# leopard-ai/betty

Measured on AMD Instinct MI355X. Metric: hypergradient-steps/sec (CG K=20, 10M inner params), higher is better.
Workload: dtype f32

## Files before the change

### betty_amd/_native.py

```python
from __future__ import annotations

import ctypes
import os
from ctypes import POINTER, c_char_p, c_double, c_float, c_int, c_int32, c_int64, c_size_t, c_void_p

_HERE = os.path.dirname(os.path.abspath(__file__))
LIB_PATH = os.environ.get("BHG_LIB") or os.path.join(_HERE, "csrc", "libbhg.so")
AB_LIB_PATH = os.environ.get("BHG_AB_LIB") or os.path.join(_HERE, "csrc", "libbhg_ab.so")

BHG_CHUNK_ELEMS = 4096
BHG_FLAT_ALIGN = 64
BHG_CG_AUTO, BHG_CG_STREAM, BHG_CG_RESIDENT = 0, 1, 2
BHG_CG_GLOBAL_CHAIN, BHG_CG_GLOBAL_UPDATE, BHG_CG_GLOBAL_DOTS = 0, 1, 2
BHG_CG_FX_BEGIN, BHG_CG_FX_CHAIN, BHG_CG_FX_GRAM, BHG_CG_FX_END = 0, 1, 2, 3


class NativeLibraryError(RuntimeError):
    """libbhg.so is missing or a call into it failed."""


class Chunk(ctypes.Structure):

    _fields_ = [
        ("flat_off", c_int64),
# ... 156 lines not shown
    "bhg_mlp_fx_slab_floats": (c_size_t, [POINTER(Mlp)]),
    "bhg_mlp_fx_scal_doubles": (c_size_t, [POINTER(Mlp)]),
    "bhg_mlp_cg_fx_phase": (
        c_int,
        [POINTER(Mlp), _PP, c_int, c_int, c_int, c_int, c_int, c_void_p, c_void_p, c_void_p, c_float, c_float, c_void_p, c_size_t,
         c_void_p, c_size_t, c_void_p],
    ),
    "bhg_mlp_neumann_fx_phase": (
        c_int,
        [POINTER(Mlp), _PP, c_int, c_int, c_int, c_int, c_int, c_void_p, c_void_p, c_void_p, c_float, c_float, c_void_p, c_size_t,
         c_void_p, c_size_t, c_void_p],
    ),
    "bhg_mlp_cg_mixed_coeff": (c_int, [POINTER(Mlp), c_void_p, c_void_p, c_float, c_void_p, c_size_t, c_void_p]),
    "bhg_mlp_timeout_flag_dev": (c_void_p, [POINTER(Mlp), c_void_p]),
    "bhg_mlp_head_j_dev": (c_void_p, [POINTER(Mlp), c_void_p, POINTER(c_int), POINTER(c_int)]),
    "bhg_mlp_stage_batch": (c_int, [POINTER(Mlp), c_void_p, c_void_p, c_void_p, c_void_p]),
    "bhg_mlp_supports_packed_prepare": (c_int, [POINTER(Mlp)]),
    "bhg_mlp_forward_packed": (c_int, [POINTER(Mlp), _PP, c_void_p, c_void_p, c_void_p, c_size_t, c_void_p]),
    "bhg_mlp_backward_packed": (c_int, [POINTER(Mlp), c_void_p, c_void_p, c_size_t, c_void_p]),
    "bhg_mwn_max_hidden": (c_int, []),
    "bhg_mlp_fd_ws_bytes": (c_size_t, [POINTER(c_int), c_int, c_int]),
    "bhg_mlp_fd_forward": (
        c_int,
        [c_void_p, c_void_p, c_int, POINTER(c_int), c_int, _PP, _PP, c_void_p, c_int, c_void_p, c_void_p, c_void_p, c_size_t, c_void_p],
    ),
    "bhg_mwn_fd_vjp": (
        c_int,
        [c_void_p, c_void_p, c_int, c_void_p, c_void_p, c_void_p, c_void_p, c_int, c_void_p, c_int, c_void_p, c_void_p, c_void_p, c_void_p,
         c_void_p],
    ),
# ... 172 lines not shown
```

### betty_amd/csrc/bhg_common.hpp

```cpp
#pragma once
#include <hip/hip_runtime.h>
#include <stdint.h>
#include <stddef.h>
#include <stdio.h>
#include <string.h>

#include "bhg.h"

namespace bhg {

constexpr int kThreads = 256;
constexpr int kWaves = kThreads / 64;
constexpr int kChunk = BHG_CHUNK_ELEMS;
constexpr int kVecPerThread = kChunk / (kThreads * 4);
constexpr int kMaxBlocks = 1024;
constexpr int kInlineT = 32;
constexpr int kWriterT = 448;

constexpr size_t kWsScal = 0;
constexpr size_t kWsPartP = 128;
constexpr size_t kWsPartR = kWsPartP + 8 * kMaxBlocks;
constexpr size_t kWsBarrier = kWsPartR + 16 * kMaxBlocks;
constexpr size_t kWsTables = kWsBarrier + 256;
inline size_t ws_bytes(int T) {
  size_t b = kWsTables + 4 * sizeof(void*) * (size_t)(T > 0 ? T : 0);
  return (b + 255) & ~(size_t)255;
}

enum { S_RR_OLD = 0, S_PHP = 1, S_ALPHA = 2, S_RR_NEW = 3, S_BETA = 4, S_PP = 5 , S_ALPHA_RING = 10 ,
       S_NPART0 = 8  };

#define BHG_DBG_KEYS(X)                                                                                                      \
  X(mlp_wsk) X(mlp_wsk_maxk) X(mlp_wsk_depth) X(mlp_wsk_lds) X(wsl_depth) X(no_nt_slabs) X(gemm_no_xpose) X(mlp_no_fast)      \
  X(mlp_tn) X(split_target) X(split_cap) X(mlp_no_head) X(gram_ksplit) X(gram_kchunk) X(proj_graw_split) X(mlp_proj)         \
  X(mlp_hoist) X(hoist_wgs) X(proj_step_alone) X(mlp_no_side) X(mlp_no_fuse) X(mlp_no_outer_all) X(neumann_side)             \
  X(hoist_staged_mink) X(proj_alpha_alone) X(proj_small_alone) X(outer_order_by_work) X(outer_no_pre) X(outer_stagger)       \
  X(mlp_no_fused_solve) X(cg_eager_p) X(cg_x_every_iter) X(neumann_p_every_iter) X(head_no_prefetch) X(cg_spin_limit)        \
  X(packed_chain) X(packed_depth) X(packed_gram) X(proj_max_ratio) X(proj_ws_cap_mb) X(alpha_in_hoist) X(graw_v2) X(wskp_ragged) X(pstep_v2) X(pstep_unroll) X(rnew_in_graw) X(graw_cols) X(lin_first) X(lin_prio) X(lin_nub) X(lin_order) X(lin_update_next) X(lin_withhold_beta) X(neumann_vnew) X(cg_rhs_direct) X(packed_prepare) X(lin_deep) X(graw_kloop) X(lin_update_in_head) X(xcd_pairs) X(headu_head_first) X(fx_ksplit) X(head_j) X(head_j_tile)
enum DbgKey : int {
#define BHG_DBG_ENUM(n) DBG_##n,
  BHG_DBG_KEYS(BHG_DBG_ENUM)
#undef BHG_DBG_ENUM
  DBG_COUNT
};
constexpr int kDbgUnset = INT32_MIN;
#ifdef BHG_AB
extern int g_dbg[DBG_COUNT];
inline bool dbg_is_set(DbgKey k) { return g_dbg[k] != kDbgUnset; }
inline int dbg(DbgKey k, int dflt) { return g_dbg[k] == kDbgUnset ? dflt : g_dbg[k]; }
#else
constexpr bool dbg_is_set(DbgKey) { return false; }
constexpr int dbg(DbgKey, int dflt) { return dflt; }
#endif
// ... 210 lines not shown
```

### betty_amd/csrc/bhg_mlp.hip

```cpp
#include <stdlib.h>


#include "bhg_common.hpp"
#include "bhg_mlp_headj.hpp"

#ifdef BHG_STAMPS
namespace bhg { __device__ unsigned long long* d_stamps = nullptr; }
#endif

namespace bhg {
namespace {
#include "mlp/gemm.inc"

#include "mlp/outer.inc"

#include "mlp/scalars.inc"

#include "mlp/head.inc"

#include "mlp/wsk.inc"

#include "mlp/wskp.inc"

inline int wsk_mode(int chain_mode, int unfused_hint) {
// ... 469 lines not shown
  int nRR, nT2;
  float* hoist;
  double* part_dot; double* pscal;
  double* part_raw;
  double* part_graw;
  float* pb0[2];
  float* pb1[2];
  unsigned long long* gran;
  float* Wf[BHG_MLP_MAX_LAYERS];
  float* Wb[BHG_MLP_MAX_LAYERS];
  float* hpk[BHG_MLP_MAX_LAYERS];
  float* dpk[BHG_MLP_MAX_LAYERS];
  float* Rhp[BHG_MLP_MAX_LAYERS];
  float* Rdp[BHG_MLP_MAX_LAYERS];
  float* hj_J; float* hj_Ap; int nT2j;
  size_t bytes;
};
inline bool headj_shape_ok(const bhg_mlp* m, const HoistPlan& hp) {
  return hp.ok && hp.lin_ok && m->L == 4 && m->dims[m->L] <= 12 && m->dims[m->L - 1] <= 512 && m->Bp == 128;
}
inline int headj_rows(int rows_valid, int C) { return (rows_valid * C + 31) & ~31; }
void carve_fused_ws(const bhg_mlp* m, void* base, FusedWs* w) {
  memset(w, 0, sizeof(*w));
  const bool head = use_head(m);
  int nrr = bias_blocks(m);
  for (int l = 0; l < m->L; ++l) nrr += outer_blocks(m, l, head);
  w->nRR = nrr;
  size_t off = 0;
  auto take = [&](size_t bytes) { void* p = base ? static_cast<char*>(base) + off : nullptr; off += (bytes + 255) & ~(size_t)255; return p; };
  w->partT1 = static_cast<double*>(take(sizeof(double) * m->Bp));
  w->partT2h = static_cast<double*>(take(sizeof(double) * m->Bp));
  w->partPP = static_cast<double*>(take(sizeof(double) * kMaxBlocks));
  w->partRR[0] = static_cast<double*>(take(sizeof(double) * 3 * nrr));
  w->partRR[1] = static_cast<double*>(take(sizeof(double) * 3 * nrr));
  int nt2 = 0;
  for (int l = 1; l + 1 < m->L; ++l) { w->t2_off[l] = nt2; nt2 += reduce_blocks(m->Bp * m->dims[l], m->dims[l]); }
// ... 19 lines not shown
    for (int l = 0; l + 1 < L; ++l) {
      w->hpk[l] = static_cast<float*>(take(sizeof(float) * Bp * m->dims[l]));
      if (l + 2 < L) w->Rhp[l] = static_cast<float*>(take(sizeof(float) * Bp * m->dims[l + 1]));
      if (l >= 1) {
        w->Wf[l] = static_cast<float*>(take(sizeof(float) * (size_t)m->dims[l + 1] * m->dims[l]));
        w->Wb[l] = static_cast<float*>(take(sizeof(float) * (size_t)m->dims[l + 1] * m->dims[l]));
        w->dpk[l] = static_cast<float*>(take(sizeof(float) * Bp * m->dims[l + 1]));
        w->Rdp[l] = static_cast<float*>(take(sizeof(float) * Bp * m->dims[l + 1]));
      }
    }
  }
  if (hj) {
    const size_t rj = (size_t)headj_rows(m->Bp, m->dims[m->L]);
    w->hj_J = static_cast<float*>(take(sizeof(float) * rj * m->dims[m->L - 2]));
    w->hj_Ap = static_cast<float*>(take(sizeof(float) * rj * m->dims[m->L - 1]));
  }
  w->bytes = off;
}

bool graw_single_on(bool packed, int Bp) { return packed && dbg(DBG_packed_gram, 1) != 0 && dbg(DBG_graw_v2, 1) != 0 && graw_batch_ok(Bp); }
bool rnew_keys_on() { return dbg(DBG_proj_small_alone, 0) == 0 && dbg(DBG_alpha_in_hoist, 1) != 0 && dbg(DBG_rnew_in_graw, 1) != 0; }

int pack_operands(const bhg_mlp* m, const FusedWs& w, hipStream_t st, bool weights_only = false) {
  PackArgs g{};
  int blk = 0;
  auto add = [&](const float* X, float* Xp, int R, int K, int kind) {
    if (g.n >= kPackMax) return false;
    g.p[g.n] = {X, Xp, R, K, kind};
    g.blk0[g.n] = blk;
    blk += pack_blocks(g.p[g.n]);
// ... 16 lines not shown
  BHG_HIP_CHECK(hipGetLastError());
  return BHG_OK;
}

int build_head_j(const bhg_mlp* m, const FusedWs& w, hipStream_t st) {
  const int L = m->L, C = m->dims[L], K = m->dims[L - 1], N = m->dims[L - 2], RA = headj_rows(m->B, C);
  BHG_REQUIRE(w.nT2j > 0 && w.hj_J && w.hj_Ap && w.Wb[L - 2], "the head_j form was planned for a net it cannot take");
  if (int rc = launch_headj_pack(m->W[L - 1], m->mask[L - 2], w.hj_Ap, m->B, C, K, RA, st)) return rc;
  WskpBuilder wb;
  WskpProb q{};
  q.Ap = w.hj_Ap; q.Bq = w.Wb[L - 2]; q.RA = RA; q.RB = N; q.K = K; q.B = m->B * C; q.nsplit = 1;
  q.out = w.hj_J;
  wb.add(q);
  wb.launch(st);
  BHG_HIP_CHECK(hipGetLastError());
  return BHG_OK;
}

#include "mlp/solve_plan.inc"
#include "mlp/chain_plan.inc"

int hoist_products(const bhg_mlp* m, const void* const* dir, const ChainMode& cm, const ChainPlan& pl, hipStream_t st, ChainState* cs) {
  const int L = m->L, Bp = m->Bp, B = m->B;
  const HoistPlan* hp = pl.hp;
  float* hbase = pl.hoist;
  HoistArgs ha{};
  HoistRedArgs ra{};
  for (int i = 0; i < hp->n; ++i) {
    const int l = hp->layer[i];
    HoistProb& q = ha.p[i];
// ... 280 lines not shown
int hoist_head(const bhg_mlp* m, const void* const* dir, const ChainMode& cm, const ChainPlan& pl, hipStream_t st, ChainState* cs) {
  const int L = m->L, Bp = m->Bp, B = m->B;
  if (cs->lin_update_pending && cs->head_j) {
    const int l = L - 1, K = m->dims[l], N = m->dims[l + 1];
    BHG_REQUIRE(cs->fuse_head && pl.cg && pl.packed && cm.ws->nT2j > 0 && !cm.rzx_acc, "k_headj was planned for a head it cannot run");
    HeadjLaunch a{};
    a.h = m->h[l]; a.W = m->W[l]; a.V = static_cast<const float*>(dir[2 * l]); a.cb = static_cast<const float*>(dir[2 * l + 1]);
    a.prob = m->prob; a.sd = m->sd; a.rd = m->Rd[l];
    a.K = K; a.C = N; a.B = B; a.rows = Bp;
    a.delta_top = (const float*)m->delta[l]; a.mask_prev = (const float*)m->mask[l - 1]; a.rd_prev = m->Rd[l - 1]; a.rd_prev_p = cm.ws->Rdp[l - 1];
    a.partT1 = cm.ws->partT1; a.rz_out = cm.ws->rz;
    a.bias2 = cs->head_fuse.bias; a.mask2 = cs->head_fuse.mask; a.addend = cs->head_fuse.addend;
    a.addend2 = pl.gp2(cm.kpar ^ 1); a.gran = cm.ws->gran;
    a.J = cm.ws->hj_J; a.Rh1 = m->Rh[l - 2]; a.K1 = m->dims[l - 1];
    a.Rh1p = cm.ws->Rhp[l - 2]; a.W2p = cm.ws->Wf[l - 1]; a.rh_out = m->Rh[l - 1];
    a.tile_shape = dbg(DBG_head_j_tile, kHeadjTile);
    const int nt = headj_tiles(Bp, K, a.tile_shape);
    if (nt <= B) { a.partT2 = cm.ws->partT2h; a.t2n = B; cs->head_j_nt = 0; }
    else { a.partT2 = cm.ws->partT2 + cm.ws->nT2; a.t2n = nt; cs->head_j_nt = nt; }
    a.ps = &cs->lin_ps; a.ps_bytes = sizeof(cs->lin_ps); a.nu = cs->lin_ps.h.update_blocks;
    if (int rc = launch_headj(a, st)) return rc;
    cs->lin_update_pending = false;
  } else if (cs->lin_update_pending) {
    const int l = L - 1, K = m->dims[l], N = m->dims[l + 1];
    BHG_REQUIRE(cs->fuse_head && pl.cg && pl.packed && N <= 12 && K <= 512, "k_headu was planned for a head it cannot run");
    HeaduArgs ha{};
    ha.Rh = (const float*)m->Rh[l - 1]; ha.h = m->h[l]; ha.W = m->W[l]; ha.V = static_cast<const float*>(dir[2 * l]);
    ha.cb = static_cast<const float*>(dir[2 * l + 1]); ha.prob = m->prob; ha.sd = m->sd; ha.rd = m->Rd[l];
    ha.K = K; ha.C = N; ha.B = B; ha.mode = HEAD_JVP;
    ha.delta_top = (const float*)m->delta[l]; ha.mask_prev = (const float*)m->mask[l - 1]; ha.rd_prev = m->Rd[l - 1];
    ha.fz = cs->head_fuse;
    ha.partT1 = cm.ws->partT1; ha.partT2h = cm.ws->partT2h; ha.rz_out = cm.ws->rz; ha.rzx_acc = cm.rzx_acc; ha.rzx_first = cm.first;
    ha.rows = Bp; ha.rd_prev_p = cm.ws->Rdp[l - 1];
    ha.addend2 = pl.gp2(cm.kpar ^ 1); ha.gran = cm.ws->gran;
// ... 521 lines not shown
  ChainState cs;
  if (pl.do_chain && pl.hp) {
    if (int rc = chain_hoisted(m, dir, cm, pl, st, &cs)) return rc;
    if (cm.stop_after_head) {
      BHG_HIP_CHECK(hipGetLastError());
      return BHG_OK;
    }
  }
  if (pl.do_chain && !pl.hp) chain_forward(m, dir, cm, pl, st, &cs);
  ChainOutputs od;
  describe_outputs(m, dir, cm, pl, &od);
  if (cs.head_j && cs.head_j_nt > 0) {
    od.aa.partT2h = nullptr;
    od.aa.nT2 = cm.ws->nT2 + cs.head_j_nt;
  }
  if (pl.do_chain && !pl.hp)
    if (int rc = chain_backward(m, dir, cm, pl, st)) return rc;

  if (pl.cg && cm.gphase == 1) {
    hipLaunchKernelGGL(k_php_local, dim3(1), dim3(kThreads), 0, st, od.aa, cm.php);
    BHG_HIP_CHECK(hipGetLastError());
    return BHG_OK;
  }
  if (pl.single) {
    if (int rc = chain_close(m, dir, cm, pl, od, st, cs)) return rc;
    BHG_HIP_CHECK(hipGetLastError());
    return BHG_OK;
  }

  const bool fork = m->L > 1 && !pl.no_side;
// ... 92 lines not shown
void* bhg_mlp_timeout_flag_dev(const bhg_mlp* m, void* fws) {
  if (!mlp_desc_ok(m) || !fws) return nullptr;
  FusedWs w;
  carve_fused_ws(m, fws, &w);
  return w.gran + 1;
}

const float* bhg_mlp_head_j_dev(const bhg_mlp* m, void* fws, int* rows, int* cols) {
  if (!mlp_desc_ok(m) || !fws) return nullptr;
  FusedWs w;
  carve_fused_ws(m, fws, &w);
  if (w.nT2j == 0) return nullptr;
  if (rows) *rows = headj_rows(m->B, m->dims[m->L]);
  if (cols) *cols = m->dims[m->L - 2];
  return w.hj_J;
}

size_t bhg_mlp_fused_ws_bytes(const bhg_mlp* m) {
  if (!mlp_desc_ok(m)) return 0;
  FusedWs w;
  carve_fused_ws(m, nullptr, &w);
  return w.bytes;
}

static int solve_common_checks(const bhg_mlp* m, const int64_t* starts, const void* fws, size_t fws_bytes) {
  if (int rc = check_mlp(m)) return rc;
  BHG_REQUIRE(bhg_mlp_supports_fused_solve(m), "fused solve needs a narrow classifier head (<= 256 classes, feature width % 4 == 0)");
  BHG_REQUIRE(starts && fws, "NULL argument");
  BHG_REQUIRE(m->partial && m->partial_floats >= bhg_mlp_partial_floats(m), "split-K scratch too small");
  BHG_REQUIRE(fws_bytes >= bhg_mlp_fused_ws_bytes(m), "fused workspace too small");
// ... 565 lines not shown
  const char* form = "unfused";
  if (fused && algo == 0)
    form = !sp.lazy ? "classic-eager" : (!sp.hoist ? "classic" : (proj_level == 0 ? "hoisted" : (proj_level == 1 ? "projected-keep-state" :
           (sp.lin ? (sp.lin_head ? "six-launch (k_wskpl .. k_headu .. k_graw)" : "six-launch-class (k_wskpl first, recurrences beside the chain)") :
            "fully-projected (k_pstep launch)"))));
  else if (fused)
    form = proj_level ? "projected-neumann (update inside k_graw)" : (sp.hoist ? "hoisted" : "classic");
  HoistPlan hp;
  hoist_plan(m, &hp);
  size_t gram = 0;
  if (hp.ok && hp.proj_ok)
    for (int l = 0; l + 1 < L; ++l) gram += (size_t)m->Bp * m->Bp * (l >= 1 ? (2 + 2 * kGramSplitMax + 6) : 2);
  const int n = snprintf(buf, buf_bytes,
                         "algo=%s keep_solution=%d fused=%d form=\"%s\" hoist=%d proj_level=%d lin=%d lin_head=%d upd_first=%d closing=%s "
                         "plan_ok=%d proj_ok=%d lin_ok=%d hoist_products=%d hoist_wgs=%d gram_floats=%zu fused_ws_bytes=%zu narrow_head=%d packed_prepare=%d "
                         "global_form=%s fx_slab_bytes=%zu fx_ws_bytes_world8=%zu head_j=%d",
                         algo == 0 ? "cg" : "neumann", keep_solution ? 1 : 0, fused ? 1 : 0, form, hoist, proj_level, lin, lin_head, upd_first, closing,
                         hp.ok ? 1 : 0, hp.proj_ok ? 1 : 0, hp.lin_ok ? 1 : 0, hp.n, hp.ok ? hp.blk0[hp.n] : 0, gram,
                         fused ? bhg_mlp_fused_ws_bytes(m) : (size_t)0, narrow_head(m) ? 1 : 0, bhg_mlp_supports_packed_prepare(m),
                         (algo == 0 && !keep_solution && bhg_mlp_fx_supported(m, 1)) ? "factor-exchange" : (fused ? "one-pass" : "sharded"),
                         sizeof(float) * bhg_mlp_fx_slab_floats(m), bhg_mlp_fx_ws_bytes(m, 8), head_j);
  BHG_REQUIRE(n > 0 && (size_t)n < buf_bytes, "output buffer too small");
  return BHG_OK;
}

#ifdef BHG_STAMPS
static unsigned long long* g_stamps_dev = nullptr;
int bhg_debug_stamps_enable(int on) {
  const size_t bytes = sizeof(unsigned long long) * bhg::kStampKernels * bhg::kStampBlocks * bhg::kStampSlots;
  if (on && !g_stamps_dev) {
    BHG_HIP_CHECK(hipMalloc(&g_stamps_dev, bytes));
  }
  if (g_stamps_dev) BHG_HIP_CHECK(hipMemset(g_stamps_dev, 0, bytes));
  unsigned long long* p = on ? g_stamps_dev : nullptr;
  BHG_HIP_CHECK(hipMemcpyToSymbol(HIP_SYMBOL(bhg::d_stamps), &p, sizeof(p)));
  return BHG_OK;
// ... 27 lines not shown
```

### betty_amd/csrc/bhg_mlp_headj.hip

```cpp
#include <stdlib.h>

#include "bhg_mlp_headj.hpp"

#ifdef BHG_STAMPS
#undef BHG_STAMP
#define BHG_STAMP(kid, slot) do { } while (0)
#endif

namespace bhg {
namespace {
#include "mlp/gemm.inc"
#include "mlp/outer.inc"
#include "mlp/scalars.inc"
#include "mlp/head.inc"
#include "mlp/wsk.inc"
#include "mlp/wskp.inc"
#include "mlp/recurrence.inc"
#include "mlp/proj.inc"
#include "mlp/pstep.inc"

struct HeadjArgs {
  const float* h; const float* W; const float* V; const float* cb; const float* prob; const float* sd; float* rd;
  int K, C, B, rows;
  const float* delta_top; const float* mask_prev; float* rd_prev; float* rd_prev_p;
  HeadFuse fz;
  double* partT1; float* rz_out;
  const float* addend2;
  const unsigned long long* gran;
  const float* J; const float* Rh1; int K1;
  const float* Rh1p; const float* W2p; double* partT2;
  int nt, nu;
  int t2n;
  alignas(64) PstepArgs ps;
};
static_assert(offsetof(HeadjArgs, ps) % 64 == 0 && sizeof(HeadjArgs) <= 3900, "kernel arguments of k_headj");

constexpr int kHjC = 12;

template <int RBLK, int CBLK>
__device__ __forceinline__ void headj_tile(const HeadjArgs& g, const int t, float* __restrict__ sPf, float* __restrict__ sD,
                                           float* __restrict__ sV, double* __restrict__ red) {
  constexpr int TR = 16 * RBLK, TC = 16 * CBLK, TCP = TC + 1;
  static_assert(kWskpWaves * TR * TCP <= kWskpLds && TR <= 32 && TC <= 32 && (TR * TC) % (64 * kWskpWaves) == 0, "four partial tiles");
  const int RA = g.rows, RB = g.K, KT = g.K1, B = g.B, C = g.C;
  const int ntm = RA / TR, ntn = RB / TC;
  int tm = t % ntm, tn = t / ntm;
  if ((ntn & 7) == 0) { const int j = t >> 3; tm = j % ntm; tn = (j / ntm) * 8 + (t & 7); }
  const int m0 = TR * tm, n0 = TC * tn;
  const int lane = threadIdx.x & 63;
  const int wave = __builtin_amdgcn_readfirstlane(threadIdx.x >> 6);
  const int li = lane & 15, lk = lane >> 4;
  const int nct = KT / 32;
  const int c0 = (int)(((int64_t)wave * nct) / kWskpWaves), c1 = (int)(((int64_t)(wave + 1) * nct) / kWskpWaves);
  const int nch_w = c1 - c0;
  f32x4 acc[RBLK][CBLK];
#pragma unroll
  for (int a = 0; a < RBLK; ++a)
#pragma unroll
    for (int b = 0; b < CBLK; ++b)
#pragma unroll
      for (int r = 0; r < 4; ++r) acc[a][b][r] = 0.f;
  constexpr int kOutPer = TR * TC / (64 * kWskpWaves);
  float e_mask[kOutPer], e_bias[kOutPer], e_add[kOutPer], e_add2[kOutPer];
// ... 6 lines not shown
    e_add[u] = g.fz.addend[idx];
    e_add2[u] = (g.addend2 ? g.addend2 : g.fz.addend)[idx];
  }
  for (int e = threadIdx.x; e < TR * C; e += 64 * kWskpWaves) {
    const int r = e / C, c = e - r * C;
    sD[r * kHjC + c] = m0 + r < B ? g.delta_top[(int64_t)(m0 + r) * C + c] : 0.f;
  }
  for (int e = threadIdx.x; e < C * TC; e += 64 * kWskpWaves) {
    const int c = e / TC, j = e % TC;
    sV[c * TC + j] = g.V[(int64_t)c * RB + n0 + j];
  }
  if (nch_w > 0) {
    const int64_t sA = (int64_t)16 * RA, sB = (int64_t)16 * RB;
    const float* gA = g.Rh1p + (int64_t)(2 * c0) * sA + (m0 + li) * 16 + 4 * lk;
    const float* gB = g.W2p + (int64_t)(2 * c0) * sB + (n0 + li) * 16 + 4 * lk;
    wskp_loop<2, RBLK, CBLK>(gA, gB, sA, sB, nch_w, acc);
  }
  float* sW = sPf + wave * (TR * TCP);
#pragma unroll
  for (int rb = 0; rb < RBLK; ++rb)
#pragma unroll
    for (int cbk = 0; cbk < CBLK; ++cbk)
#pragma unroll
      for (int r = 0; r < 4; ++r) sW[(16 * rb + 4 * lk + r) * TCP + 16 * cbk + li] = acc[rb][cbk][r];
  __syncthreads();
  const float beta = g.addend2 ? poll_beta(g.gran) : 0.f;
  double t2 = 0.0;
#pragma unroll
  for (int u = 0; u < kOutPer; ++u) {
    const int e = threadIdx.x + 64 * kWskpWaves * u;
    const int row = e / TC, col = e % TC;
// ... 7 lines not shown
    v += ad;
    v = (v + e_bias[u]) * e_mask[u];
    v = m < B ? v : 0.f;
    g.fz.rh_out[idx] = v;
    float dv = 0.f;
    for (int c = 0; c < C; ++c) dv += sD[row * kHjC + c] * sV[c * TC + col];
    if (m < B) t2 += (double)dv * (double)v;
  }
  t2 = wave_sum(t2);
  if (lane == 0) red[wave] = t2;
  __syncthreads();
  if (threadIdx.x == 0) {
    double s = 0.0;
#pragma unroll
    for (int w = 0; w < kWskpWaves; ++w) s += red[w];
    g.partT2[t] = 2.0 * s;
    for (int z = t + g.nt; z < g.t2n; z += g.nt) g.partT2[z] = 0.0;
  }
}

template <int U, int TS>
__global__ __launch_bounds__(256) void k_headj(HeadjArgs g) {
  static_assert(64 * kWskpWaves == 256, "the tiles run in the head launch's workgroups");
  const int bx = (int)blockIdx.x;
  if (bx >= g.rows + g.nt) { pstep_body<U, (int)offsetof(HeadjArgs, ps), false>(bx - g.rows - g.nt); return; }
  if (bx >= g.rows) {
    __shared__ float sPf[kWskpLds];
    __shared__ float sD[32 * kHjC], sV[kHjC * 32];
    __shared__ double red[kWskpWaves];
    if constexpr (TS == 0) headj_tile<2, 2>(g, bx - g.rows, sPf, sD, sV, red);
    else headj_tile<2, 1>(g, bx - g.rows, sPf, sD, sV, red);
    return;
  }
  const float* __restrict__ Rh = nullptr; const float* __restrict__ h = g.h; const float* __restrict__ W = g.W;
  const float* __restrict__ V = g.V; const float* __restrict__ cb = g.cb; const float* __restrict__ prob = g.prob;
  const float* __restrict__ sd = g.sd; float* __restrict__ rd = g.rd;
  const int K = g.K, C = g.C, B = g.B;
  constexpr int mode = HEAD_JVP;
  const int64_t* __restrict__ labels = nullptr; float* __restrict__ aux = nullptr; const float* __restrict__ delta_top = g.delta_top;
  const float* __restrict__ mask_prev = g.mask_prev; float* __restrict__ rd_prev = g.rd_prev;
  const HeadFuse fz = g.fz;
  double* __restrict__ partT1 = g.partT1; double* __restrict__ partT2h = nullptr; float* __restrict__ rz_out = g.rz_out;
  double* __restrict__ rzx_acc = nullptr; const int rzx_first = 0; float* __restrict__ rd_prev_p = g.rd_prev_p;
  const float* __restrict__ lazy_addend2 = g.addend2;
  const float lazy_beta = g.addend2 ? poll_beta(g.gran) : 0.f;
  const float* __restrict__ hj_J = g.J; const float* __restrict__ hj_Rh1 = g.Rh1; const int hj_K1 = g.K1;
  constexpr bool HAS_RH = true, FUSED = true, PF = true;
  constexpr int JMAX = 3;
  (void)Rh; (void)labels; (void)aux; (void)rzx_acc; (void)rzx_first;
#define BHG_HEAD_B (bx)
#define BHG_HEAD_ROWS (g.rows)
#define BHG_HEAD_LAZY 1
#define BHG_HEAD_J 1
#include "mlp/head_body.inc"
#undef BHG_HEAD_B
#undef BHG_HEAD_ROWS
#undef BHG_HEAD_LAZY
#undef BHG_HEAD_J
}

__global__ __launch_bounds__(256) void k_headj_pack(const float* __restrict__ W3, const float* __restrict__ mask2, float* __restrict__ Ap,
                                                    const int B, const int C, const int K, const int RA) {
  const int64_t idx = (int64_t)blockIdx.x * 256 + threadIdx.x;
  const int64_t total = (int64_t)RA * K / 4;
  if (idx >= total) return;
// ... 1 lines not shown
  const int64_t rr = idx >> 2;
  const int r = (int)(rr % RA), kb = (int)(rr / RA);
  const int k = 16 * kb + 4 * c4;
  f32x4 v = {0.f, 0.f, 0.f, 0.f};
  if (r < B * C) {
    const int b = r / C, c = r - b * C;
    const f32x4 w = *reinterpret_cast<const f32x4*>(W3 + (int64_t)c * K + k);
    const f32x4 mk = *reinterpret_cast<const f32x4*>(mask2 + (int64_t)b * K + k);
#pragma unroll
    for (int j = 0; j < 4; ++j) v[j] = w[j] * mk[j];
  }
  *reinterpret_cast<f32x4*>(Ap + idx * 4) = v;
}
}

int headj_tiles(int rows, int K, int shape) { return (rows / 32) * (K / (shape == 0 ? 32 : 16)); }

int launch_headj(const HeadjLaunch& a, hipStream_t st) {
  BHG_REQUIRE(a.C >= 1 && a.C <= kHjC && a.K >= 32 && a.K <= 512 && a.K % 32 == 0 && a.K1 >= 32 && a.K1 % 32 == 0 && a.rows % 32 == 0 &&
              a.B >= 1 && a.B <= a.rows, "k_headj was planned for a head it cannot run");
  BHG_REQUIRE(a.ps && a.ps_bytes == sizeof(PstepArgs) && a.nu >= 0, "the update blocks' arguments do not match this build");
  BHG_REQUIRE(a.J && a.Rh1 && a.Rh1p && a.W2p && a.rh_out && a.partT2 && a.addend && a.bias2 && a.mask2 && a.rd_prev && a.delta_top &&
              a.mask_prev, "NULL argument");
  HeadjArgs g{};
  g.h = a.h; g.W = a.W; g.V = a.V; g.cb = a.cb; g.prob = a.prob; g.sd = a.sd; g.rd = a.rd;
  g.K = a.K; g.C = a.C; g.B = a.B; g.rows = a.rows;
  g.delta_top = a.delta_top; g.mask_prev = a.mask_prev; g.rd_prev = a.rd_prev; g.rd_prev_p = a.rd_prev_p;
  g.fz = HeadFuse{nullptr, 0, a.rows * a.K, a.bias2, a.mask2, a.rh_out, a.addend};
  g.partT1 = a.partT1; g.rz_out = a.rz_out; g.addend2 = a.addend2; g.gran = a.gran;
  g.J = a.J; g.Rh1 = a.Rh1; g.K1 = a.K1; g.Rh1p = a.Rh1p; g.W2p = a.W2p; g.partT2 = a.partT2;
  g.nt = headj_tiles(a.rows, a.K, a.tile_shape); g.nu = a.nu; g.t2n = a.t2n;
  BHG_REQUIRE(a.t2n >= g.nt, "fewer T2h slots than tiles");
  memcpy(&g.ps, a.ps, sizeof(PstepArgs));
  const dim3 grid(a.rows + g.nt + g.nu);
  const size_t lds = (size_t)a.K * sizeof(float);
#ifdef BHG_AB
  if (a.tile_shape == 0) hipLaunchKernelGGL((k_headj<4, 0>), grid, dim3(256), lds, st, g); else
#endif
  hipLaunchKernelGGL((k_headj<4, 1>), grid, dim3(256), lds, st, g);
  return BHG_OK;
}

int launch_headj_pack(const float* W3, const float* mask2, float* Ap, int B, int C, int K, int RA, hipStream_t st) {
  BHG_REQUIRE(W3 && mask2 && Ap && B >= 1 && C >= 1 && K % 16 == 0 && RA % 32 == 0 && RA >= B * C, "bad arguments");
  const int64_t total = (int64_t)RA * K / 4;
  hipLaunchKernelGGL(k_headj_pack, dim3((unsigned)((total + 255) / 256)), dim3(256), 0, st, W3, mask2, Ap, B, C, K, RA);
  return BHG_OK;
}

}
```

### betty_amd/csrc/bhg_mlp_headj.hpp

```cpp
#pragma once
#include <stddef.h>

#include "bhg_common.hpp"

namespace bhg {

struct HeadjLaunch {
  const float* h; const float* W; const float* V; const float* cb; const float* prob; const float* sd; float* rd;
  int K, C, B, rows;
  const float* delta_top; const float* mask_prev; float* rd_prev; float* rd_prev_p;
  double* partT1; float* rz_out;
  const float* bias2; const float* mask2;
  const float* addend; const float* addend2; const unsigned long long* gran;
  const float* J;
  const float* Rh1;
  int K1;
  const float* Rh1p; const float* W2p;
  float* rh_out;
  double* partT2; int t2n;
  int tile_shape;
  const void* ps; size_t ps_bytes; int nu;
};
constexpr int kHeadjTile = 1;
int headj_tiles(int rows, int K, int shape);
int launch_headj(const HeadjLaunch& a, hipStream_t st);

int launch_headj_pack(const float* W3, const float* mask2, float* Ap, int B, int C, int K, int RA, hipStream_t st);

}
```

### betty_amd/csrc/mlp/chain_plan.inc

```

struct ChainMode {
  int mode;
  void* const* out;
  float* fa; float* fb; float* fd;
  const int64_t* starts;
  float alpha, shift, out_scale;
  int apply_out;
  FusedWs* ws;
  const double* partRR_old; int nRR_old;
  const double* partPP; int nPP;
  double* partRR_new;
  double* scal;
  float cg_alpha;
  int kpar;
  int x_mode;
  int first;
  int lazy;
  double* rzx_acc;
  int skip_outputs;
  int gemm_mode;
  const SolvePlan* sp;
  const BetaArgs* beta; int beta_blocks;
  int stop_after_head;
  int gphase; double* php; double inv_world;
// ... 26 lines not shown
  float* rh0_slot(int k) const { return (k & 1) ? hoist + hp->rh0alt_off : rh0; }
  float* gp1(int par) const { return hoist + (par ? hp->gp1alt_off : hp->g_off[hp->gf[1]]); }
  float* gp2(int par) const { return hoist + (par ? hp->gp2alt_off : hp->g_off[hp->gf[L - 2]]); }
  int gram_slabs(int K) const { return gram_in_chain ? 1 : gram_ksplit(K); }
};

struct ChainState {
  HeadFuse head_fuse{};
  bool fuse_head = false;
  PstepArgs lin_ps{};
  int lin_nu = 0, lin_U = 4;
  bool lin_update_pending = false;
  bool sd_in_chain = false;
  bool head_j = false;
  int head_j_nt = 0;
};

int plan_chain(const bhg_mlp* m, const ChainMode& cm, ChainPlan* p) {
  const int L = m->L;
  *p = ChainPlan{};
  p->L = L;
  p->rho2 = cm.mode == FUSE_NONE ? m->ridge2 : 0.f;
  const bool cg = p->cg = cm.mode == FUSE_CG;
  const bool no_side_env = dbg(DBG_mlp_no_side, 0) != 0;
  p->no_fuse = dbg(DBG_mlp_no_fuse, 0) != 0;
  p->no_outer_all = dbg(DBG_mlp_no_outer_all, 0) != 0;
  const bool neumann_side = dbg(DBG_neumann_side, 0) != 0;
  p->single = cg || (cm.mode == FUSE_NEUMANN && !neumann_side && !p->no_outer_all);
  p->no_side = no_side_env || p->single;
  p->head = use_head(m);
// ... 40 lines not shown
```

### betty_amd/csrc/mlp/solve_plan.inc

```

inline bool mlp_desc_ok(const bhg_mlp* m) { return m && m->L >= 1 && m->L <= BHG_MLP_MAX_LAYERS && m->Bp > 0; }
inline bool mlp_desc_tiled(const bhg_mlp* m) { return mlp_desc_ok(m) && m->Bp % kTM == 0; }

struct SolvePlan {
  bool fused;
  HoistPlan hp;
  bool lazy;
  bool hoist;
  int proj_level;
  bool packed, graw_single;
  bool rnew, vnew;
  int nt;
  bool lin, lin_head, head_j, upd_first;
  const char* closing;
};

void plan_solve(const bhg_mlp* m, int algo, bool keep_solution, bool global, SolvePlan* sp) {
  memset(sp, 0, sizeof(*sp));
  sp->closing = "k_outer_all";
  sp->fused = bhg_mlp_supports_fused_solve(m) != 0;
  if (!sp->fused) return;
  HoistPlan& hp = sp->hp;
  const bool head = use_head(m);
  sp->nt = m->L + (head ? 1 : 0);
  if (algo == 0) {
    sp->lazy = global || dbg(DBG_cg_eager_p, 0) == 0;
    if (sp->lazy && hoist_mode() != 0) hoist_plan(m, &hp);
    sp->hoist = sp->lazy && hp.ok;
    sp->proj_level = (!sp->hoist || !hp.proj_ok || proj_mode() == 0 || global) ? 0 : ((proj_mode() == 9 || keep_solution) ? 1 : 2);
  } else {
    const bool want_proj = !keep_solution && proj_mode() != 0 && hoist_mode() != 0;
    if (hoist_mode() == 2 || want_proj) hoist_plan(m, &hp);
    sp->hoist = hp.ok;
    sp->proj_level = (want_proj && hp.ok && hp.proj_ok && head) ? 1 : 0;
  }
  sp->packed = hp.ok && dbg(DBG_packed_chain, 1) != 0;
  sp->graw_single = graw_single_on(sp->packed, m->Bp);
  sp->rnew = algo == 0 && sp->graw_single && sp->proj_level >= 2 && rnew_keys_on();
  sp->vnew = algo == 1 && sp->proj_level && sp->graw_single && m->L >= 3 && dbg(DBG_neumann_vnew, 1) != 0;
  sp->lin = algo == 0 && sp->proj_level == 2 && hp.lin_ok && sp->rnew && sp->nt <= 16 && proj_step_merged() && dbg(DBG_pstep_v2, 1) != 0 &&
            dbg(DBG_lin_first, 1) != 0;
  sp->lin_head = sp->lin && m->L == 4 && dbg(DBG_lin_update_next, 1) != 0 && dbg(DBG_lin_update_in_head, 1) != 0 && dbg(DBG_lin_nub, 0) == 0 &&
                 m->dims[m->L] <= 12 && m->dims[m->L - 1] <= 512 && dbg(DBG_head_no_prefetch, 0) == 0;
  sp->head_j = sp->lin_head && headj_shape_ok(m, hp) && dbg(DBG_head_j, 1) != 0;
  sp->upd_first = sp->lin && m->L > 4;
  if (sp->proj_level >= 1) sp->closing = graw_batch_ok(m->Bp) ? (m->Bp == 128 ? "k_graw" : "k_grawk") : "k_hoist+k_proj_update";
}
```

### include/bhg.h

```cpp
#ifndef BHG_H_
#define BHG_H_

#include <stddef.h>
#include <stdint.h>

#ifdef __cplusplus
extern "C" {
#endif

#define BHG_VERSION 1
#define BHG_CHUNK_ELEMS 4096
#define BHG_FLAT_ALIGN 64

#define BHG_OK 0
#define BHG_ERR_ARG (-1)
#define BHG_ERR_HIP (-2)
#define BHG_ERR_WS (-3)
#define BHG_ERR_CAPACITY (-4)

typedef struct bhg_chunk {
  int64_t flat_off;
  int64_t src_off;
  int32_t tensor;
  int32_t len;
// ... 164 lines not shown
int64_t bhg_mlp_hoist_launches(void);
int64_t bhg_mlp_proj_iterations(void);
int64_t bhg_mlp_lin_launches(void);
int bhg_mlp_neumann_mixed_coeff(const bhg_mlp* m, const void* const* v_last, const int64_t* labels, float* coeff,
                                float alpha, int K, int projected, void* fws, size_t fws_bytes, void* stream);

int bhg_mlp_stage_batch(const bhg_mlp* m, const float* x, const int64_t* y, int64_t* labels, void* stream);
int bhg_mlp_supports_packed_prepare(const bhg_mlp* m);
int bhg_mlp_forward_packed(const bhg_mlp* m, const void* const* bias, const int64_t* labels, float* ce, void* fws, size_t fws_bytes,
                           void* stream);
int bhg_mlp_backward_packed(const bhg_mlp* m, const int64_t* labels, void* fws, size_t fws_bytes, void* stream);

void* bhg_mlp_timeout_flag_dev(const bhg_mlp* m, void* fws);

const float* bhg_mlp_head_j_dev(const bhg_mlp* m, void* fws, int* rows, int* cols);

int bhg_mwn_max_hidden(void);
int bhg_mwn_forward(const float* ce, int B, const float* w1, const float* b1, const float* w2, const float* b2, int H, float* s,
                    float* sd, void* stream);
int bhg_mwn_backward(const float* ce, const float* coeff, int B, const float* w1, const float* b1, const float* w2, const float* b2,
                     int H, float scale, float* gw1, float* gb1, float* gw2, float* gb2, void* stream);

int bhg_mlp_plan_describe(const bhg_mlp* m, int algo, int keep_solution, char* buf, size_t buf_bytes);

int bhg_copy2d(float* dst, int64_t ldd, const float* src, int64_t lds, int64_t rows, int64_t cols, void* stream);

size_t bhg_bn_ws_bytes(int C);
int bhg_bn_plan(int N, int C, int HW, char* buf, size_t buf_bytes);
int bhg_bn_backward_vjp(const float* x, const float* gy, const float* a, const float* gamma, const float* mean, const float* invstd,
                        const float* b, const float* c, int N, int C, int HW, float* dx, float* dgy, float* dgamma, void* ws,
// ... 40 lines not shown
```

Measured before the change: 776.7.

## Use finer 16x16 head_j tiles with paired atomic T2h reduction

Adds a third head_j tile shape (16x16) that is chosen automatically when the tile count fits within batch slots. Tiles run first in the launch and pair-reduce their T2 partial sums by atomically adding into a double-buffered per-parity T2h array. Head rows clear the other parity's buffer, replacing the separate zeroing of extra slots. The aim is more, smaller tiles for better parallelism in the head launch, at the cost of double atomics, an extra memset at setup and more workspace.

```diff
diff --git a/betty_amd/_native.py b/betty_amd/_native.py
--- a/betty_amd/_native.py
+++ b/betty_amd/_native.py
@@ -194,6 +194,7 @@
     "bhg_mlp_cg_mixed_coeff": (c_int, [POINTER(Mlp), c_void_p, c_void_p, c_float, c_void_p, c_size_t, c_void_p]),
     "bhg_mlp_timeout_flag_dev": (c_void_p, [POINTER(Mlp), c_void_p]),
     "bhg_mlp_head_j_dev": (c_void_p, [POINTER(Mlp), c_void_p, POINTER(c_int), POINTER(c_int)]),
+    "bhg_mlp_head_j_t2h_dev": (c_void_p, [POINTER(Mlp), c_void_p, POINTER(c_int)]),
     "bhg_mlp_stage_batch": (c_int, [POINTER(Mlp), c_void_p, c_void_p, c_void_p, c_void_p]),
     "bhg_mlp_supports_packed_prepare": (c_int, [POINTER(Mlp)]),
     "bhg_mlp_forward_packed": (c_int, [POINTER(Mlp), _PP, c_void_p, c_void_p, c_void_p, c_size_t, c_void_p]),
diff --git a/betty_amd/csrc/bhg_common.hpp b/betty_amd/csrc/bhg_common.hpp
--- a/betty_amd/csrc/bhg_common.hpp
+++ b/betty_amd/csrc/bhg_common.hpp
@@ -36,7 +36,7 @@
   X(mlp_hoist) X(hoist_wgs) X(proj_step_alone) X(mlp_no_side) X(mlp_no_fuse) X(mlp_no_outer_all) X(neumann_side)             \
   X(hoist_staged_mink) X(proj_alpha_alone) X(proj_small_alone) X(outer_order_by_work) X(outer_no_pre) X(outer_stagger)       \
   X(mlp_no_fused_solve) X(cg_eager_p) X(cg_x_every_iter) X(neumann_p_every_iter) X(head_no_prefetch) X(cg_spin_limit)        \
-  X(packed_chain) X(packed_depth) X(packed_gram) X(proj_max_ratio) X(proj_ws_cap_mb) X(alpha_in_hoist) X(graw_v2) X(wskp_ragged) X(pstep_v2) X(pstep_unroll) X(rnew_in_graw) X(graw_cols) X(lin_first) X(lin_prio) X(lin_nub) X(lin_order) X(lin_update_next) X(lin_withhold_beta) X(neumann_vnew) X(cg_rhs_direct) X(packed_prepare) X(lin_deep) X(graw_kloop) X(lin_update_in_head) X(xcd_pairs) X(headu_head_first) X(fx_ksplit) X(head_j) X(head_j_tile)
+  X(packed_chain) X(packed_depth) X(packed_gram) X(proj_max_ratio) X(proj_ws_cap_mb) X(alpha_in_hoist) X(graw_v2) X(wskp_ragged) X(pstep_v2) X(pstep_unroll) X(rnew_in_graw) X(graw_cols) X(lin_first) X(lin_prio) X(lin_nub) X(lin_order) X(lin_update_next) X(lin_withhold_beta) X(neumann_vnew) X(cg_rhs_direct) X(packed_prepare) X(lin_deep) X(graw_kloop) X(lin_update_in_head) X(xcd_pairs) X(headu_head_first) X(fx_ksplit) X(head_j) X(head_j_tile) X(head_j_stages4) X(head_j_tiles_first)
 enum DbgKey : int {
 #define BHG_DBG_ENUM(n) DBG_##n,
   BHG_DBG_KEYS(BHG_DBG_ENUM)
diff --git a/betty_amd/csrc/bhg_mlp.hip b/betty_amd/csrc/bhg_mlp.hip
--- a/betty_amd/csrc/bhg_mlp.hip
+++ b/betty_amd/csrc/bhg_mlp.hip
@@ -507,12 +507,17 @@
   float* Rhp[BHG_MLP_MAX_LAYERS];
   float* Rdp[BHG_MLP_MAX_LAYERS];
   float* hj_J; float* hj_Ap; int nT2j;
+  double* hj_t2h[2];
   size_t bytes;
 };
 inline bool headj_shape_ok(const bhg_mlp* m, const HoistPlan& hp) {
   return hp.ok && hp.lin_ok && m->L == 4 && m->dims[m->L] <= 12 && m->dims[m->L - 1] <= 512 && m->Bp == 128;
 }
 inline int headj_rows(int rows_valid, int C) { return (rows_valid * C + 31) & ~31; }
+inline int head_j_tile(const bhg_mlp* m) {
+  const int want = dbg(DBG_head_j_tile, 2);
+  return (want == 0 || want == 1) ? want : headj_tile_shape(m->Bp, m->dims[m->L - 1], m->B);
+}
 void carve_fused_ws(const bhg_mlp* m, void* base, FusedWs* w) {
   memset(w, 0, sizeof(*w));
   const bool head = use_head(m);
@@ -562,6 +567,8 @@
     const size_t rj = (size_t)headj_rows(m->Bp, m->dims[m->L]);
     w->hj_J = static_cast<float*>(take(sizeof(float) * rj * m->dims[m->L - 2]));
     w->hj_Ap = static_cast<float*>(take(sizeof(float) * rj * m->dims[m->L - 1]));
+    w->hj_t2h[0] = static_cast<double*>(take(sizeof(double) * 2 * m->Bp));
+    w->hj_t2h[1] = w->hj_t2h[0] ? w->hj_t2h[0] + m->Bp : nullptr;
   }
   w->bytes = off;
 }
@@ -608,6 +615,7 @@
   wb.add(q);
   wb.launch(st);
   BHG_HIP_CHECK(hipGetLastError());
+  if (head_j_tile(m) == 2) BHG_HIP_CHECK(hipMemsetAsync(w.hj_t2h[0], 0, sizeof(double) * 2 * m->Bp, st));
   return BHG_OK;
 }
 
@@ -918,10 +926,13 @@
     a.addend2 = pl.gp2(cm.kpar ^ 1); a.gran = cm.ws->gran;
     a.J = cm.ws->hj_J; a.Rh1 = m->Rh[l - 2]; a.K1 = m->dims[l - 1];
     a.Rh1p = cm.ws->Rhp[l - 2]; a.W2p = cm.ws->Wf[l - 1]; a.rh_out = m->Rh[l - 1];
-    a.tile_shape = dbg(DBG_head_j_tile, kHeadjTile);
+    a.tile_shape = head_j_tile(m);
+    a.stages4 = dbg(DBG_head_j_stages4, 0); a.tiles_first = dbg(DBG_head_j_tiles_first, 1);
     const int nt = headj_tiles(Bp, K, a.tile_shape);
-    if (nt <= B) { a.partT2 = cm.ws->partT2h; a.t2n = B; cs->head_j_nt = 0; }
-    else { a.partT2 = cm.ws->partT2 + cm.ws->nT2; a.t2n = nt; cs->head_j_nt = nt; }
+    a.partT2 = cm.ws->partT2 + cm.ws->nT2; a.t2n = nt;
+    if (a.tile_shape == 2) { a.t2pair = cm.ws->hj_t2h[cm.kpar]; a.t2clear = cm.ws->hj_t2h[cm.kpar ^ 1]; cs->head_j_nt = 0; cs->head_j_t2h = a.t2pair; }
+    else if (nt <= B) { a.partT2 = cm.ws->partT2h; a.t2n = B; cs->head_j_nt = 0; }
+    else cs->head_j_nt = nt;
     a.ps = &cs->lin_ps; a.ps_bytes = sizeof(cs->lin_ps); a.nu = cs->lin_ps.h.update_blocks;
     if (int rc = launch_headj(a, st)) return rc;
     cs->lin_update_pending = false;
@@ -1473,6 +1484,7 @@
     od.aa.partT2h = nullptr;
     od.aa.nT2 = cm.ws->nT2 + cs.head_j_nt;
   }
+  if (cs.head_j && cs.head_j_t2h) od.aa.partT2h = cs.head_j_t2h;
   if (pl.do_chain && !pl.hp)
     if (int rc = chain_backward(m, dir, cm, pl, st)) return rc;
 
@@ -1595,6 +1607,15 @@
   if (rows) *rows = headj_rows(m->B, m->dims[m->L]);
   if (cols) *cols = m->dims[m->L - 2];
   return w.hj_J;
+}
+
+double* bhg_mlp_head_j_t2h_dev(const bhg_mlp* m, void* fws, int* doubles) {
+  if (!mlp_desc_ok(m) || !fws) return nullptr;
+  FusedWs w;
+  carve_fused_ws(m, fws, &w);
+  if (w.nT2j == 0) return nullptr;
+  if (doubles) *doubles = 2 * m->Bp;
+  return w.hj_t2h[0];
 }
 
 size_t bhg_mlp_fused_ws_bytes(const bhg_mlp* m) {
@@ -2190,12 +2211,12 @@
   const int n = snprintf(buf, buf_bytes,
                          "algo=%s keep_solution=%d fused=%d form=\"%s\" hoist=%d proj_level=%d lin=%d lin_head=%d upd_first=%d closing=%s "
                          "plan_ok=%d proj_ok=%d lin_ok=%d hoist_products=%d hoist_wgs=%d gram_floats=%zu fused_ws_bytes=%zu narrow_head=%d packed_prepare=%d "
-                         "global_form=%s fx_slab_bytes=%zu fx_ws_bytes_world8=%zu head_j=%d",
+                         "global_form=%s fx_slab_bytes=%zu fx_ws_bytes_world8=%zu head_j=%d head_j_tile=%d",
                          algo == 0 ? "cg" : "neumann", keep_solution ? 1 : 0, fused ? 1 : 0, form, hoist, proj_level, lin, lin_head, upd_first, closing,
                          hp.ok ? 1 : 0, hp.proj_ok ? 1 : 0, hp.lin_ok ? 1 : 0, hp.n, hp.ok ? hp.blk0[hp.n] : 0, gram,
                          fused ? bhg_mlp_fused_ws_bytes(m) : (size_t)0, narrow_head(m) ? 1 : 0, bhg_mlp_supports_packed_prepare(m),
                          (algo == 0 && !keep_solution && bhg_mlp_fx_supported(m, 1)) ? "factor-exchange" : (fused ? "one-pass" : "sharded"),
-                         sizeof(float) * bhg_mlp_fx_slab_floats(m), bhg_mlp_fx_ws_bytes(m, 8), head_j);
+                         sizeof(float) * bhg_mlp_fx_slab_floats(m), bhg_mlp_fx_ws_bytes(m, 8), head_j, sp.head_j_tile);
   BHG_REQUIRE(n > 0 && (size_t)n < buf_bytes, "output buffer too small");
   return BHG_OK;
 }
diff --git a/betty_amd/csrc/bhg_mlp_headj.hip b/betty_amd/csrc/bhg_mlp_headj.hip
--- a/betty_amd/csrc/bhg_mlp_headj.hip
+++ b/betty_amd/csrc/bhg_mlp_headj.hip
@@ -31,13 +31,14 @@
   const float* Rh1p; const float* W2p; double* partT2;
   int nt, nu;
   int t2n;
+  double* t2clear;
   alignas(64) PstepArgs ps;
 };
 static_assert(offsetof(HeadjArgs, ps) % 64 == 0 && sizeof(HeadjArgs) <= 3900, "kernel arguments of k_headj");
 
 constexpr int kHjC = 12;
 
-template <int RBLK, int CBLK>
+template <int RBLK, int CBLK, int D, bool PAIR>
 __device__ __forceinline__ void headj_tile(const HeadjArgs& g, const int t, float* __restrict__ sPf, float* __restrict__ sD,
                                            float* __restrict__ sV, double* __restrict__ red) {
   constexpr int TR = 16 * RBLK, TC = 16 * CBLK, TCP = TC + 1;
@@ -47,6 +48,12 @@
   int tm = t % ntm, tn = t / ntm;
   if ((ntn & 7) == 0) { const int j = t >> 3; tm = j % ntm; tn = (j / ntm) * 8 + (t & 7); }
   const int m0 = TR * tm, n0 = TC * tn;
+  if (m0 >= B) {
+    for (int e = threadIdx.x; e < TR * TC; e += 64 * kWskpWaves) g.fz.rh_out[(int64_t)(m0 + e / TC) * RB + n0 + (e % TC)] = 0.f;
+    if (!PAIR && threadIdx.x == 0)
+      for (int z = t; z < g.t2n; z += g.nt) g.partT2[z] = 0.0;
+    return;
+  }
   const int lane = threadIdx.x & 63;
   const int wave = __builtin_amdgcn_readfirstlane(threadIdx.x >> 6);
   const int li = lane & 15, lk = lane >> 4;
@@ -83,7 +90,7 @@
     const int64_t sA = (int64_t)16 * RA, sB = (int64_t)16 * RB;
     const float* gA = g.Rh1p + (int64_t)(2 * c0) * sA + (m0 + li) * 16 + 4 * lk;
     const float* gB = g.W2p + (int64_t)(2 * c0) * sB + (n0 + li) * 16 + 4 * lk;
-    wskp_loop<2, RBLK, CBLK>(gA, gB, sA, sB, nch_w, acc);
+    wskp_loop<D, RBLK, CBLK>(gA, gB, sA, sB, nch_w, acc);
   }
   float* sW = sPf + wave * (TR * TCP);
 #pragma unroll
@@ -121,24 +128,32 @@
     double s = 0.0;
 #pragma unroll
     for (int w = 0; w < kWskpWaves; ++w) s += red[w];
-    g.partT2[t] = 2.0 * s;
-    for (int z = t + g.nt; z < g.t2n; z += g.nt) g.partT2[z] = 0.0;
-  }
-}
-
-template <int U, int TS>
+    if constexpr (PAIR) {
+      atomicAdd(g.partT2 + tn * (ntm / 2) + (tm >> 1), 2.0 * s);
+    } else {
+      g.partT2[t] = 2.0 * s;
+      for (int z = t + g.nt; z < g.t2n; z += g.nt) g.partT2[z] = 0.0;
+    }
+  }
+}
+
+template <int U, int TS, int D, bool TF>
 __global__ __launch_bounds__(256) void k_headj(HeadjArgs g) {
   static_assert(64 * kWskpWaves == 256, "the tiles run in the head launch's workgroups");
   const int bx = (int)blockIdx.x;
   if (bx >= g.rows + g.nt) { pstep_body<U, (int)offsetof(HeadjArgs, ps), false>(bx - g.rows - g.nt); return; }
-  if (bx >= g.rows) {
+  if (TF ? bx < g.nt : bx >= g.rows) {
     __shared__ float sPf[kWskpLds];
     __shared__ float sD[32 * kHjC], sV[kHjC * 32];
     __shared__ double red[kWskpWaves];
-    if constexpr (TS == 0) headj_tile<2, 2>(g, bx - g.rows, sPf, sD, sV, red);
-    else headj_tile<2, 1>(g, bx - g.rows, sPf, sD, sV, red);
+    const int t = TF ? bx : bx - g.rows;
+    if constexpr (TS == 0) headj_tile<2, 2, D, false>(g, t, sPf, sD, sV, red);
+    else if constexpr (TS == 1) headj_tile<2, 1, D, false>(g, t, sPf, sD, sV, red);
+    else headj_tile<1, 1, D, true>(g, t, sPf, sD, sV, red);
     return;
   }
+  const int hrow = TF ? bx - g.nt : bx;
+  if (TS == 2 && threadIdx.x == 0) g.t2clear[hrow] = 0.0;
   const float* __restrict__ Rh = nullptr; const float* __restrict__ h = g.h; const float* __restrict__ W = g.W;
   const float* __restrict__ V = g.V; const float* __restrict__ cb = g.cb; const float* __restrict__ prob = g.prob;
   const float* __restrict__ sd = g.sd; float* __restrict__ rd = g.rd;
@@ -155,7 +170,7 @@
   constexpr bool HAS_RH = true, FUSED = true, PF = true;
   constexpr int JMAX = 3;
   (void)Rh; (void)labels; (void)aux; (void)rzx_acc; (void)rzx_first;
-#define BHG_HEAD_B (bx)
+#define BHG_HEAD_B (hrow)
 #define BHG_HEAD_ROWS (g.rows)
 #define BHG_HEAD_LAZY 1
 #define BHG_HEAD_J 1
@@ -187,7 +202,7 @@
 }
 }
 
-int headj_tiles(int rows, int K, int shape) { return (rows / 32) * (K / (shape == 0 ? 32 : 16)); }
+int headj_tiles(int rows, int K, int shape) { return (rows / (shape == 2 ? 16 : 32)) * (K / (shape == 0 ? 32 : 16)); }
 
 int launch_headj(const HeadjLaunch& a, hipStream_t st) {
   BHG_REQUIRE(a.C >= 1 && a.C <= kHjC && a.K >= 32 && a.K <= 512 && a.K % 32 == 0 && a.K1 >= 32 && a.K1 % 32 == 0 && a.rows % 32 == 0 &&
@@ -203,14 +218,24 @@
   g.partT1 = a.partT1; g.rz_out = a.rz_out; g.addend2 = a.addend2; g.gran = a.gran;
   g.J = a.J; g.Rh1 = a.Rh1; g.K1 = a.K1; g.Rh1p = a.Rh1p; g.W2p = a.W2p; g.partT2 = a.partT2;
   g.nt = headj_tiles(a.rows, a.K, a.tile_shape); g.nu = a.nu; g.t2n = a.t2n;
-  BHG_REQUIRE(a.t2n >= g.nt, "fewer T2h slots than tiles");
+  BHG_REQUIRE(a.tile_shape >= 0 && a.tile_shape <= 2, "unknown tile shape");
+  if (a.tile_shape == 2) {
+    BHG_REQUIRE(a.t2pair && a.t2clear && a.t2pair != a.t2clear && g.nt / 2 <= a.B, "16 x 16 tiles: one T2h slot per pair, in a buffer per parity");
+    g.partT2 = a.t2pair; g.t2clear = a.t2clear;
+  } else {
+    BHG_REQUIRE(a.t2n >= g.nt, "fewer T2h slots than tiles");
+  }
   memcpy(&g.ps, a.ps, sizeof(PstepArgs));
   const dim3 grid(a.rows + g.nt + g.nu);
   const size_t lds = (size_t)a.K * sizeof(float);
 #ifdef BHG_AB
-  if (a.tile_shape == 0) hipLaunchKernelGGL((k_headj<4, 0>), grid, dim3(256), lds, st, g); else
+  if (a.tile_shape == 0) hipLaunchKernelGGL((k_headj<4, 0, 2, false>), grid, dim3(256), lds, st, g);
+  else if (a.tile_shape == 2 && a.stages4) hipLaunchKernelGGL((k_headj<4, 2, 4, false>), grid, dim3(256), lds, st, g);
+  else if (a.tile_shape == 2 && !a.tiles_first) hipLaunchKernelGGL((k_headj<4, 2, 2, false>), grid, dim3(256), lds, st, g);
+  else
 #endif
-  hipLaunchKernelGGL((k_headj<4, 1>), grid, dim3(256), lds, st, g);
+  if (a.tile_shape == 2) hipLaunchKernelGGL((k_headj<4, 2, 2, true>), grid, dim3(256), lds, st, g);
+  else hipLaunchKernelGGL((k_headj<4, 1, 2, false>), grid, dim3(256), lds, st, g);
   return BHG_OK;
 }
 
diff --git a/betty_amd/csrc/bhg_mlp_headj.hpp b/betty_amd/csrc/bhg_mlp_headj.hpp
--- a/betty_amd/csrc/bhg_mlp_headj.hpp
+++ b/betty_amd/csrc/bhg_mlp_headj.hpp
@@ -18,11 +18,19 @@
   const float* Rh1p; const float* W2p;
   float* rh_out;
   double* partT2; int t2n;
+  double* t2pair; double* t2clear;
   int tile_shape;
+  int stages4;
+  int tiles_first;
   const void* ps; size_t ps_bytes; int nu;
 };
 constexpr int kHeadjTile = 1;
+constexpr int kHeadjFineMax = 192;
 int headj_tiles(int rows, int K, int shape);
+inline int headj_tile_shape(int rows, int K, int B) {
+  const int nt = (rows / 16) * (K / 16);
+  return (nt / 2 <= B && nt <= kHeadjFineMax) ? 2 : kHeadjTile;
+}
 int launch_headj(const HeadjLaunch& a, hipStream_t st);
 
 int launch_headj_pack(const float* W3, const float* mask2, float* Ap, int B, int C, int K, int RA, hipStream_t st);
diff --git a/betty_amd/csrc/mlp/chain_plan.inc b/betty_amd/csrc/mlp/chain_plan.inc
--- a/betty_amd/csrc/mlp/chain_plan.inc
+++ b/betty_amd/csrc/mlp/chain_plan.inc
@@ -64,6 +64,7 @@
   bool sd_in_chain = false;
   bool head_j = false;
   int head_j_nt = 0;
+  double* head_j_t2h = nullptr;
 };
 
 int plan_chain(const bhg_mlp* m, const ChainMode& cm, ChainPlan* p) {
diff --git a/betty_amd/csrc/mlp/solve_plan.inc b/betty_amd/csrc/mlp/solve_plan.inc
--- a/betty_amd/csrc/mlp/solve_plan.inc
+++ b/betty_amd/csrc/mlp/solve_plan.inc
@@ -12,12 +12,14 @@
   bool rnew, vnew;
   int nt;
   bool lin, lin_head, head_j, upd_first;
+  int head_j_tile;
   const char* closing;
 };
 
 void plan_solve(const bhg_mlp* m, int algo, bool keep_solution, bool global, SolvePlan* sp) {
   memset(sp, 0, sizeof(*sp));
   sp->closing = "k_outer_all";
+  sp->head_j_tile = -1;
   sp->fused = bhg_mlp_supports_fused_solve(m) != 0;
   if (!sp->fused) return;
   HoistPlan& hp = sp->hp;
@@ -43,6 +45,7 @@
   sp->lin_head = sp->lin && m->L == 4 && dbg(DBG_lin_update_next, 1) != 0 && dbg(DBG_lin_update_in_head, 1) != 0 && dbg(DBG_lin_nub, 0) == 0 &&
                  m->dims[m->L] <= 12 && m->dims[m->L - 1] <= 512 && dbg(DBG_head_no_prefetch, 0) == 0;
   sp->head_j = sp->lin_head && headj_shape_ok(m, hp) && dbg(DBG_head_j, 1) != 0;
+  sp->head_j_tile = sp->head_j ? head_j_tile(m) : -1;
   sp->upd_first = sp->lin && m->L > 4;
   if (sp->proj_level >= 1) sp->closing = graw_batch_ok(m->Bp) ? (m->Bp == 128 ? "k_graw" : "k_grawk") : "k_hoist+k_proj_update";
 }
diff --git a/include/bhg.h b/include/bhg.h
--- a/include/bhg.h
+++ b/include/bhg.h
@@ -202,6 +202,7 @@
 void* bhg_mlp_timeout_flag_dev(const bhg_mlp* m, void* fws);
 
 const float* bhg_mlp_head_j_dev(const bhg_mlp* m, void* fws, int* rows, int* cols);
+double* bhg_mlp_head_j_t2h_dev(const bhg_mlp* m, void* fws, int* doubles);
 
 int bhg_mwn_max_hidden(void);
 int bhg_mwn_forward(const float* ce, int B, const float* w1, const float* b1, const float* w2, const float* b2, int H, float* s,
```

After: 791.9 (median of 6 runs). +1.9%, better.
